# DoHoonKim8/halo2-lasso

Hardware: AMD Instinct MI355X
Metric: lasso_prove_time_ms (lower is better)
Workload: dtype u256 (BN254 Fr/Fq, 8x u32 Montgomery); 1 GPU; 2^24 AND Lasso lookup (32-bit operands, 4 chunks of 8+8 bits); lookups_per_proof=16777216, pcs=multilinear KZG (BN254), proof_bytes=64256, parallelism=1 GPU

## Files before the change

halo2-lasso_amd/_ffi.py:

```python
import ctypes as C
import os

_HERE = os.path.dirname(os.path.abspath(__file__))
LIB_PATH = os.path.join(_HERE, "liblasso_hip.so")

LH_OK = 0
LH_ERR_INVALID_SUMCHECK, LH_ERR_INVALID_PCS_PARAM, LH_ERR_INVALID_PCS_OPEN = -1, -2, -3
LH_ERR_INVALID_SNARK, LH_ERR_SERIALIZATION, LH_ERR_TRANSCRIPT, LH_ERR_DEVICE, LH_ERR_ARG = -4, -5, -6, -7, -8
LH_SC_EVALUATIONS, LH_SC_COEFFICIENTS = 0, 1
LH_SC_MAX_TERMS, LH_SC_MAX_FACTORS = 48, 4
LH_LASSO_MAX_CHUNKS, LH_LASSO_MAX_MEMORIES, LH_LASSO_MAX_TERMS = 8, 16, 16
LH_SUBTABLE_IDENTITY, LH_SUBTABLE_AND, LH_SUBTABLE_XOR, LH_SUBTABLE_OR, LH_SUBTABLE_EQ, LH_SUBTABLE_LTU = 0, 1, 2, 3, 4, 5
LH_SUBTABLE_CUSTOM_BASE, LH_SUBTABLE_CUSTOM_MAX, LH_SUBTABLE_CUSTOM_MAX_BITS = 0x100, 64, 20
LH_LASSO_NUM_PHASES = 9
LH_LOGUP_MAX_LOOKUPS, LH_LOGUP_MAX_WIDTH, LH_LOGUP_MAX_TABLE_VARS = 8, 8, 24
LH_LOGUP_COL_FR, LH_LOGUP_COL_U32 = 0, 1
LH_MEMCHECK_MAX_INIT_VARS = 24
LH_SPARK_MAX_DIMS, LH_SPARK_MAX_DIM_VARS = 3, 24
LH_BD_COLUMN_FR, LH_BD_COLUMN_U32 = 0, 1


class lh_fr(C.Structure):
    _fields_ = [("l", C.c_uint64 * 4)]

# ... 84 lines not shown


_AG_CB = C.CFUNCTYPE(C.c_int, C.c_void_p, C.c_void_p, C.c_void_p, C.c_size_t)
_AGD_CB = C.CFUNCTYPE(C.c_int, C.c_void_p, C.c_void_p, C.c_void_p, C.c_size_t, C.c_void_p)
LH_RCCL_UNIQUE_ID_BYTES = 128


class lh_comm(C.Structure):
    _fields_ = [("rank", C.c_int), ("size", C.c_int), ("user", C.c_void_p), ("all_gather", _AG_CB),
                ("all_gather_device", _AGD_CB)]


class lh_debug_sort_slab(C.Structure):
    _fields_ = [("d_keys_in", C.c_void_p), ("d_keys_out", C.c_void_p), ("d_vals_in", C.c_void_p), ("d_vals_out", C.c_void_p),
                ("n", C.c_size_t), ("bits", C.c_uint32), ("first_bit", C.c_uint32)]


class lh_debug_u32_args(C.Structure):
    _fields_ = [("d_cols", C.POINTER(C.c_void_p)), ("lens", C.POINTER(C.c_size_t)), ("w", C.POINTER(lh_fr)),
                ("count", C.c_size_t), ("d_weights", C.c_void_p), ("n", C.c_size_t),
                ("d_fr", C.POINTER(C.c_void_p)), ("w_fr", C.POINTER(lh_fr)), ("num_fr", C.c_size_t),
                ("r0", lh_fr), ("r1", lh_fr), ("d_out", C.c_void_p), ("out_host", C.POINTER(lh_fr)),
                ("taken", C.POINTER(C.c_int))]


LH_U32_OPS = ("inner_products_small", "inner_products_small_half", "inner_products_small_quads", "inner_products_quads",
              "lincomb_mixed", "lincomb_fold_small", "lincomb_bind2", "sc_round_u32_bind2", None,
              "quad_sums")


# ... 172 lines not shown
    "lh_hyrax_open": (C.c_int, [_P, _P, _SZ, _SZ, _P, _SZ, C.POINTER(lh_fr), C.POINTER(lh_transcript)]),
    "lh_hyrax_batch_open": (C.c_int, [_P, _P, _SZ, _SZ, _SZ, C.POINTER(_P), _SZ, C.POINTER(lh_fr), _SZ,
                                      C.POINTER(lh_evaluation), _SZ, C.POINTER(lh_transcript)]),
    "lh_hyrax_verify": (C.c_int, [_P, _SZ, _SZ, C.POINTER(lh_g1), C.POINTER(lh_fr), _SZ, C.POINTER(lh_fr),
                                  C.POINTER(lh_transcript)]),
    "lh_hyrax_batch_verify": (C.c_int, [_P, _SZ, _SZ, _SZ, C.POINTER(lh_g1), _SZ, C.POINTER(lh_fr), _SZ,
                                        C.POINTER(lh_evaluation), _SZ, C.POINTER(lh_transcript)]),
    "lh_debug_jit_source": (C.c_int, [C.POINTER(C.c_uint32), _SZ, C.c_uint32, C.c_uint32, C.c_int, C.c_char_p, _SZ,
                                      C.POINTER(_SZ)]),
    "lh_debug_sort_pairs": (C.c_int, [_P, C.c_int, C.POINTER(lh_debug_sort_slab), _SZ]),
    "lh_debug_lasso_counters": (C.c_int, [_P, C.POINTER(_P), _SZ, _SZ, _SZ, C.POINTER(_P), C.POINTER(_P), C.POINTER(_P),
                                          C.POINTER(_P)]),
    "lh_debug_sort_plan": (C.c_int, [_SZ, C.c_uint, C.c_int, C.POINTER(C.c_uint), C.POINTER(C.c_uint), C.POINTER(_SZ)]),
    "lh_debug_msm_plan": (C.c_int, [_SZ, C.POINTER(_SZ), C.POINTER(C.c_uint32), C.POINTER(C.c_uint32), C.c_int, C.c_int,
                                    C.POINTER(C.c_uint64), C.POINTER(_SZ)]),
    "lh_debug_u32_columns": (C.c_int, [_P, C.c_int, C.POINTER(lh_debug_u32_args)]),
    "lh_debug_lasso_subtable_read": (C.c_int, [_P, C.c_uint32, C.c_uint32, _P, _SZ, _P]),
    "lh_keccak_transcript_hash_io": (C.c_int, [C.POINTER(lh_transcript), C.POINTER(lh_hash_transcript)]),
    "lh_brakedown_setup": (C.c_int, [_P, _SZ, C.c_int, C.c_char_p, C.POINTER(_P)]),
    "lh_brakedown_derive": (C.c_int, [_SZ, C.c_int, C.POINTER(_P)]),
    "lh_brakedown_param_info": (C.c_int, [_P, C.POINTER(_SZ), C.POINTER(_SZ), C.POINTER(_SZ), C.POINTER(_SZ),
                                          C.POINTER(_SZ)]),
    "lh_brakedown_trim": (C.c_int, [_P, _SZ]),
    "lh_brakedown_param_free": (None, [_P]),
    "lh_brakedown_encode": (C.c_int, [_P, C.POINTER(lh_fr), C.POINTER(lh_fr)]),
    "lh_brakedown_commit": (C.c_int, [_P, _P, _P, _SZ, C.POINTER(_P)]),
    "lh_brakedown_batch_commit": (C.c_int, [_P, _P, C.POINTER(_P), _SZ, _SZ, C.POINTER(_P)]),
    "lh_brakedown_commit_columns": (C.c_int, [_P, _P, C.POINTER(_P), C.POINTER(C.c_int), C.POINTER(_SZ), _SZ, C.POINTER(_P)]),
    "lh_brakedown_comm_root": (C.c_int, [_P, C.c_char_p]),
    "lh_brakedown_comm_rows": (C.c_int, [_P, _P, _P]),
# ... 98 lines not shown
```

halo2-lasso_amd/csrc/capi.cpp:

```cpp
#include "host.hpp"
#include "brakedown.hpp"
#include <memory>

using namespace lh;

struct lh_ctx {
  Ctx c;
};
struct lh_srs {
  Srs s;
};
struct lh_mkzg_vp {
  VerifierParams* p;
};
struct lh_usrs {
  USrs s;
};
struct lh_zm_vp {
  ZmVerifierParams* p;
};
struct lh_ukzg_vp {
  UkzgVerifierParams* p;
};
struct lh_ipa_param {
// ... 2231 lines not shown
  NEED(out);
  NEED(num_subs);
  LH_REQUIRE(num_jobs >= 1 && num_jobs <= 48, LH_ERR_ARG, "debug msm plan: 1 .. 48 jobs");
  Ctx c;
  c.is_helper = helper != 0;
  std::vector<MsmJob> jobs;
  G1Affine second;
  for (size_t j = 0; j < num_jobs; j++) {
    LH_REQUIRE(bits[j] >= 1 && bits[j] <= (kinds[j] ? 32u : 254u), LH_ERR_ARG, "debug msm plan: bad width");
    MsmJob jb{nullptr, kinds[j] != 0, nullptr, n[j]};
    jb.known_bits = bits[j];
    if (kinds[j] >= 4) jb.pack_shift = kinds[j], jb.out_second = &second;
    jobs.push_back(jb);
  }
  *num_subs = msm_plan_shape(c, jobs.data(), num_jobs, via_prepare != 0, out);
  LH_CATCH
}

lh_status lh_debug_u32_columns(lh_ctx* ctx, int op, const lh_debug_u32_args* a) {
  LH_TRY NEED_CTX(ctx);
  NEED(a);
  Ctx& c = ctx->c;
  LH_REQUIRE((op >= LH_U32_INNER_PRODUCTS_SMALL && op <= LH_U32_SC_ROUND_BIND2) || op == LH_U32_QUAD_SUMS, LH_ERR_ARG,
             "debug u32 columns: unknown operation");
  LH_REQUIRE(a->n >= 1 && a->n < ((size_t)1 << 31), LH_ERR_ARG, "debug u32 columns: n must be in [1, 2^31)");
  const bool one_col = op == LH_U32_INNER_PRODUCTS_SMALL_QUADS || op == LH_U32_SC_ROUND_BIND2;
  const bool has_lens = op == LH_U32_INNER_PRODUCTS_QUADS || op == LH_U32_QUAD_SUMS || op == LH_U32_LINCOMB_MIXED ||
                        op == LH_U32_LINCOMB_FOLD_SMALL || op == LH_U32_LINCOMB_BIND2;
  const bool has_w = op == LH_U32_LINCOMB_MIXED || op == LH_U32_LINCOMB_FOLD_SMALL || op == LH_U32_LINCOMB_BIND2;
  const bool quads = op == LH_U32_INNER_PRODUCTS_SMALL_QUADS || op == LH_U32_INNER_PRODUCTS_QUADS || op == LH_U32_QUAD_SUMS ||
// ... 121 lines not shown
```

halo2-lasso_amd/csrc/dev.hpp:

```cpp
#pragma once
#include <hip/hip_runtime_api.h>
#include <stdint.h>
#include <stdarg.h>
#include <stdio.h>
#include <functional>
#include <memory>
#include <string>
#include <vector>
#include <utility>
#include <stdexcept>

#include "../../include/lasso_hip.h"
#include "ec.cuh"

namespace lh {

struct Error : std::exception {
  int code;
  std::string msg;
  Error(int c, std::string m) : code(c), msg(std::move(m)) {}
  const char* what() const noexcept override { return msg.c_str(); }
};

void set_last_error(const char* msg);
// ... 346 lines not shown
void k_lasso_rw_leaves(Ctx&, const uint32_t* dim, const uint32_t* e, const uint32_t* ts, size_t n,
                       const Fr& gamma, const Fr& gamma2, const Fr& tau, Fr* rs, Fr* ws);
void k_lasso_rw_leaves_up(Ctx&, const uint32_t* dim, const uint32_t* e, const uint32_t* ts, size_t n, const Fr& gamma,
                          const Fr& gamma2, const Fr& tau, Fr* rs, Fr* ws, Fr* rs_up, Fr* ws_up);
constexpr int LASSO_RW_BATCH_MAX = 8;
struct LassoRwBatch {
  const uint32_t *dim[LASSO_RW_BATCH_MAX], *e[LASSO_RW_BATCH_MAX], *ts[LASSO_RW_BATCH_MAX];
  Fr *rs[LASSO_RW_BATCH_MAX], *ws[LASSO_RW_BATCH_MAX], *rs_up[LASSO_RW_BATCH_MAX], *ws_up[LASSO_RW_BATCH_MAX];
};
void k_lasso_rw_leaves_batch(Ctx&, const LassoRwBatch& p, size_t num_memories, size_t n, bool up, const Fr& gamma,
                             const Fr& gamma2, const Fr& tau);
void k_lasso_if_leaves(Ctx&, int subtable, uint32_t chunk_bits, const uint32_t* final_cts, size_t m,
                       const Fr& gamma, const Fr& gamma2, const Fr& tau, Fr* init, Fr* fin, const uint32_t* tab = nullptr);
void k_or_u32(Ctx&, const uint32_t* const* cols, size_t count, size_t n, uint32_t* out_host);
void k_fill_u32(Ctx&, uint32_t* out, uint32_t value, size_t n);
void k_pack_u32(Ctx&, const uint32_t* a, const uint32_t* b, uint32_t shift, size_t n, uint32_t* out);
void k_delta_u32(Ctx&, const uint32_t* col, size_t len, size_t half, uint64_t offset, uint32_t* out_lo, uint32_t* out_hi);
void k_lasso_counters(Ctx&, const uint32_t* const* dims, size_t cc, size_t n, size_t m, uint32_t* const* read_ts,
                      uint32_t* const* final_cts, uint32_t* const* keep_sorted = nullptr, uint32_t* const* keep_index = nullptr);
void k_cs_partition(Ctx&, const uint32_t* const* dims, size_t cc, size_t n, size_t m, unsigned rho, unsigned j, unsigned hi_bits,
                    uint32_t* const* sidx, uint32_t* const* send, uint32_t* start_host, bool* bad_out);
void k_cs_rank(Ctx&, const uint32_t* const* recv, const size_t* n_recv, size_t cc, unsigned hi_bits, unsigned a_bits, size_t m_loc,
               uint32_t* const* ret, uint32_t* counts);
void k_cs_scatter(Ctx&, const uint32_t* const* back, const uint32_t* const* sidx, size_t cc, size_t n, uint32_t* const* read_ts);
void k_cs_final(Ctx&, const uint32_t* all_counts, size_t cc, size_t m, unsigned rho, size_t m_loc, uint32_t* const* final_cts);
void k_lasso_subtable_read(Ctx&, int subtable, uint32_t chunk_bits, const uint32_t* dim, size_t n, uint32_t* e,
                           const uint32_t* tab = nullptr);
struct LassoG {
  uint32_t num_terms;
  Fr coeff[LH_LASSO_MAX_TERMS];
  uint8_t nfac[LH_LASSO_MAX_TERMS];
// ... 294 lines not shown
  const uint32_t* keys_in;
  uint32_t* keys_out;
  const uint32_t* vals_in;
  uint32_t* vals_out;
  size_t n;
  unsigned bits;
  unsigned first_bit = 0;
};
void sort_pairs_u32(Ctx&, const uint32_t* keys_in, uint32_t* keys_out, const uint32_t* vals_in, uint32_t* vals_out, size_t n,
                    unsigned bits, unsigned first_bit = 0);
void sort_pairs_u32_batched(Ctx&, const SortSlab* slabs, size_t count);
void sort_pairs_u64(Ctx&, const uint64_t* keys_in, uint64_t* keys_out, const uint32_t* vals_in, uint32_t* vals_out, size_t n,
                    unsigned bits);
void sort_plan(size_t n, unsigned bits, size_t key_bytes, unsigned* passes, unsigned rb[8], size_t* temp_bytes);

struct MsmJob {
  const void* scalars;
  bool scalars_u32;
  const G1Affine* bases;
  size_t n;
  int derived_parent = -1;
  const uint32_t* d_table = nullptr;
  const uint32_t* d_order = nullptr;
  uint32_t table_in_bits = 0, table_out_bits = 0;
  const uint32_t* sorted_scalars = nullptr;
  const uint32_t* sorted_index = nullptr;
  uint32_t pack_shift = 0;
  G1Affine* out_second = nullptr;
  uint32_t known_bits = 0;
  const G1Affine* win_table = nullptr;
  uint32_t win_table_c = 0, win_table_W = 0;
};
constexpr uint32_t MSM_PACK_MAX_BITS = 20;
constexpr size_t MSM_PACK_MIN_POINTS_PER_BUCKET = 8;
Ctx& ctx_helper(Ctx&);
void open_precommit_cancel(Ctx&);
void open_precommit_release(Ctx&);
uint32_t msm_window_bits(size_t n);
void k_msm_window_table(Ctx&, const G1Affine* bases, size_t n, uint32_t cbits, uint32_t W, G1Affine* out);
bool msm_batch(Ctx&, const MsmJob* jobs, size_t num_jobs, G1Affine* out_host, const std::function<void()>* overlap = nullptr,
               const std::function<void(bool on_aux)>* acc_queued = nullptr);
struct MsmPrepared;
struct MsmPreparedDelete {
  void operator()(MsmPrepared*) const;
};
typedef std::unique_ptr<MsmPrepared, MsmPreparedDelete> MsmPreparedPtr;
// ... 8 lines not shown
```

halo2-lasso_amd/csrc/kernels_poly.hip:

```cpp
#include <hip/hip_runtime.h>
#include <string.h>
#include <algorithm>
#include "dev.hpp"
#include "ff_host.hpp"
#include "launch.cuh"
#include "reduce.cuh"
#include "resident.cuh"
#include "wide.cuh"

namespace lh {

__global__ void fr_from_u64_kernel(const uint64_t* __restrict__ in, size_t n, Fr* __restrict__ out) {
  GSTRIDE(i, n) out[i] = from_u64<FrParams>(in[i]);
}
__global__ void fr_from_u32_kernel(const uint32_t* __restrict__ in, size_t n, Fr* __restrict__ out) {
  GSTRIDE(i, n) out[i] = from_u64<FrParams>(in[i]);
}
__global__ void fr_to_repr_kernel(const Fr* __restrict__ in, size_t n, Fr* __restrict__ out) {
  GSTRIDE(i, n) out[i] = from_mont(in[i]);
}
__global__ void fr_from_repr_kernel(const Fr* __restrict__ in, size_t n, Fr* __restrict__ out) {
  GSTRIDE(i, n) out[i] = to_mont(in[i]);
}
void k_fr_from_u64(Ctx& c, const uint64_t* in, size_t n, Fr* out) {
// ... 1486 lines not shown
  GSTRIDE(i, half) {
    const uint64_t lo = i < len ? col[i] : 0u, hi = i + half < len ? col[i + half] : 0u;
    const uint64_t v = hi + offset - lo;
    if (out_hi) {
      out_lo[i] = (uint32_t)(v & 0xffffu);
      out_hi[i] = (uint32_t)(v >> 16);
    } else {
      out_lo[i] = (uint32_t)v;
    }
  }
}
void k_delta_u32(Ctx& c, const uint32_t* col, size_t len, size_t half, uint64_t offset, uint32_t* out_lo, uint32_t* out_hi) {
  if (half)
    hipLaunchKernelGGL(delta_u32_kernel, grid_for(half), 256, 0, c.stream, col, len, half, offset, out_lo, out_hi);
}
__global__ void pack_u32_kernel(const uint32_t* __restrict__ a, const uint32_t* __restrict__ b, uint32_t shift, size_t n,
                                uint32_t* __restrict__ out) {
  GSTRIDE(i, n) out[i] = a[i] | (b[i] << shift);
}
void k_pack_u32(Ctx& c, const uint32_t* a, const uint32_t* b, uint32_t shift, size_t n, uint32_t* out) {
  if (n) hipLaunchKernelGGL(pack_u32_kernel, grid_for(n), 256, 0, c.stream, a, b, shift, n, out);
}

__global__ void lasso_rw_leaves_kernel(const uint32_t* __restrict__ dim, const uint32_t* __restrict__ e,
                                       const uint32_t* __restrict__ ts, size_t n, Fr gamma_r, Fr gamma2_r, Fr one_r, Fr tau,
                                       Fr* __restrict__ rs, Fr* __restrict__ ws) {
  const Fr one = Fr::one();
  GSTRIDE(i, n) {
    Wide t = Wide::zero();
    wide_mac(t, gamma2_r, dim[i]);
    wide_mac(t, gamma_r, e[i]);
    wide_mac(t, one_r, ts[i]);
    Fr h = sub(wide_redc(t), tau);
    rs[i] = h;
    ws[i] = add(h, one);
  }
}
// ... 150 lines not shown
```

halo2-lasso_amd/csrc/lasso.cpp:

```cpp
#include <algorithm>
#include <chrono>
#include "host.hpp"

namespace lh {

static double now_ms() {
  using namespace std::chrono;
  return duration<double, std::milli>(steady_clock::now().time_since_epoch()).count();
}

void lasso_write_commitments(Transcript& tr, const std::vector<HG1>& comms, size_t chunks) {
  LH_REQUIRE(chunks >= 1 && comms.size() % chunks == 0 && comms.size() / chunks < 64, LH_ERR_ARG,
             "lasso: too many commitments for the identity mask");
  for (size_t k = 0; 63 * k < comms.size(); k++) {
    uint64_t mask = 0;
    for (size_t i = 0; i < 63 && 63 * k + i < comms.size(); i++)
      if (comms[63 * k + i].is_identity()) mask |= (uint64_t)1 << i;
    tr.write_field_element(HFr::from_u64(mask));
  }
  for (const HG1& cm : comms)
    if (!cm.is_identity()) tr.write_commitment(cm);
}

std::vector<HG1> lasso_read_commitments(Transcript& tr, size_t count, size_t chunks) {
// ... 449 lines not shown
    own++;
  }
  plan.second.assign(cc, HG1());
  std::vector<HG1>& second = plan.second;
  {
    std::vector<uint32_t>& ors = count_ors;
    std::vector<const uint32_t*> cols(fcs.begin(), fcs.end());
    const bool pack_on = c.opt.lasso_pack_ts != 0;
    if (!ors_known && pack_on && cc >= 2 && N >= ((size_t)1 << 12)) k_or_u32(c, cols.data(), cc, M, ors.data());
    for (size_t j = 0; j < cc; j++) {
      if (shared(j)) continue;
      const bool next = j + 1 < cc && !shared(j + 1);
      const uint32_t b0 = std::max(bit_length(ors[j]), 4u), b1 = next ? bit_length(ors[j + 1]) : 0;
      if (ors[j] && next && ors[j + 1] && b0 + b1 <= MSM_PACK_MAX_BITS &&
          N >= ((size_t)MSM_PACK_MIN_POINTS_PER_BUCKET << (b0 + b1))) {
        uint32_t* packed = c.arena.alloc_n<uint32_t>(N);
        k_pack_u32(c, rts[j], rts[j + 1], b0, N, packed);
        add_job(lay.read_ts(j), packed, true, N);
        jobs.back().known_bits = b0 + b1;
        jobs.back().pack_shift = b0;
        jobs.back().out_second = (G1Affine*)&second[j + 1];
        plan.second_of.push_back(j + 1);
        c.route.v[RouteStats::PACKED_TS]++;
        j++;
      } else {
        add_job(lay.read_ts(j), rts[j], true, N);
        jobs.back().known_bits = bit_length(ors[j]);
      }
    }
  }
  SubtableOrders& orders = *w.tables;
  for (size_t i = 0; i < alpha; i++)
    if (tb.memory_subtable[i] != LH_SUBTABLE_IDENTITY) {
      add_job(lay.E(i), E[i], true, N);
      bool derive = l <= 20 && tb.memory_subtable[i] != LH_SUBTABLE_EQ;
// ... 483 lines not shown
```

halo2-lasso_amd/csrc/msm.hip:

```cpp
#include <hip/hip_runtime.h>
#include <algorithm>
#include <exception>
#include <functional>
#include <thread>
#include <vector>
#include <mutex>
#include "dev.hpp"
#include "ff_host.hpp"

namespace lh {

constexpr int MSM_MAX_JOBS = 48;
constexpr uint32_t SENTINEL = 0xffffffffu;
constexpr uint32_t SKIP_IDX = 0x7fffffffu;

struct MsmJobDev {
  const void* scalars;
  const G1Affine* bases;
  uint32_t is_u32;
  uint32_t n;
  uint32_t c, W;
  uint32_t key_base;
  uint32_t entry_base;
  uint32_t win_stride;
  uint32_t is_signed;
  uint32_t seg_base;
  uint32_t seg_per_win;
  uint32_t seg_size;
  uint32_t win_base;
  uint32_t presorted;
// ... 3 lines not shown
  uint32_t share_base;
  uint32_t two_level;
  uint32_t grp_base;
  uint32_t sum_per_win;
  uint32_t merged;
};
constexpr uint32_t KEY_BLOCK_BITS = 10;
struct MsmPlanDev {
  int num_jobs;
  const uint8_t* job_of_block;
  MsmJobDev job[MSM_MAX_JOBS];
};

__global__ void msm_or_limbs_kernel(MsmPlanDev plan, uint32_t* __restrict__ or_out ) {
  const MsmJobDev& jb = plan.job[blockIdx.y];
  uint32_t acc[8];
#pragma unroll
  for (int k = 0; k < 8; k++) acc[k] = 0;
  if (jb.is_u32) {
    for (size_t i = (size_t)blockIdx.x * blockDim.x + threadIdx.x; i < jb.n; i += (size_t)gridDim.x * blockDim.x)
      acc[0] |= ((const uint32_t*)jb.scalars)[i];
  } else {
    for (size_t i = (size_t)blockIdx.x * blockDim.x + threadIdx.x; i < jb.n; i += (size_t)gridDim.x * blockDim.x) {
      Fr s = from_mont(((const Fr*)jb.scalars)[i]);
#pragma unroll
      for (int k = 0; k < 8; k++) acc[k] |= s.l[k];
    }
  }
  __shared__ uint32_t lds_or[8];
  if (threadIdx.x < 8) lds_or[threadIdx.x] = 0;
// ... 6 lines not shown
  }
  __syncthreads();
  if (threadIdx.x < 8 && lds_or[threadIdx.x]) atomicOr(&or_out[blockIdx.y * 8 + threadIdx.x], lds_or[threadIdx.x]);
}

__global__ void msm_presorted_kernel(uint32_t key_base, const uint32_t* __restrict__ sorted_scalars,
                                     const uint32_t* __restrict__ sorted_index, size_t n, uint32_t* __restrict__ skey,
                                     uint32_t* __restrict__ sidx) {
  for (size_t p = (size_t)blockIdx.x * blockDim.x + threadIdx.x; p < n; p += (size_t)gridDim.x * blockDim.x) {
    const uint32_t d = sorted_scalars[p];
    skey[p] = key_base + (d ? d - 1u : 0u);
    sidx[p] = d ? sorted_index[p] : SKIP_IDX;
  }
}

__global__ void msm_emit_kernel(MsmPlanDev plan, uint32_t* __restrict__ keys, uint32_t* __restrict__ vals) {
  const MsmJobDev& jb = plan.job[blockIdx.y];
  if (jb.presorted) return;
  const uint32_t c = jb.c, mask = (1u << c) - 1u;
  for (size_t i = (size_t)blockIdx.x * blockDim.x + threadIdx.x; i < jb.n; i += (size_t)gridDim.x * blockDim.x) {
    uint32_t limb[8];
#pragma unroll
    for (int k = 0; k < 8; k++) limb[k] = 0;
    if (jb.is_u32) {
      limb[0] = ((const uint32_t*)jb.scalars)[i];
    } else {
      Fr s = from_mont(((const Fr*)jb.scalars)[i]);
#pragma unroll
      for (int k = 0; k < 8; k++) limb[k] = s.l[k];
    }
    const int nlimbs = jb.is_u32 ? 1 : 8;
    uint64_t buf = 0;
    int have = 0;
    uint32_t w = 0;
    uint32_t carry = 0;
    const uint32_t half = 1u << (c - 1);
    auto emit = [&](uint32_t raw) {
      uint32_t d = raw + carry, neg = 0;
      if (jb.is_signed) {
// ... 435 lines not shown
namespace {
struct MsmSub {
  std::vector<size_t> idx;
  MsmPlanDev plan;
  std::vector<uint32_t> bits, sort_bits;
  std::vector<char> derived, slab;
  size_t num_derived = 0, max_entries = 0, small_entries = 0, max_n = 0, nbuckets = 0, nsegs = 0, nwins = 0, ngroups = 0, nblocks = 0;
  size_t nchunks = 0;
  uint32_t nshares = 0, K = 0, seg_size = 0;
  bool plain_reduce = false;
  double total_pts = 0, full_pts = 0;
  uint32_t *ukey = nullptr, *uidx = nullptr, *skey = nullptr, *sidx = nullptr, *lvl_cnt = nullptr, *ckey = nullptr;
  G1Xyzz *buckets = nullptr, *seg_out = nullptr, *seg_t = nullptr, *grp_out = nullptr, *cpt = nullptr;
  G1Xyzz* win_out = nullptr;
  uint8_t* h_tab = nullptr;
  std::vector<G1Xyzz> wins;
  size_t pin_bytes() const { return ((size_t)nshares * sizeof(G1Xyzz) + nblocks + 255) & ~(size_t)255; }
};

struct MsmShape {
  uint32_t c, W, sort_bits;
  size_t entries, buckets;
};
MsmShape msm_job_shape(const MsmJob& in, uint32_t bits, bool derived) {
  MsmShape s;
  s.c = pick_window(in.n ? in.n : 1, bits ? bits : 1);
  if (in.pack_shift) s.c = std::max<uint32_t>(bits, 4);
  const bool is_signed = !in.scalars_u32;
  if (is_signed && s.c < 2) s.c = 2;
  s.W = bits ? ((is_signed ? bits + 1 : bits) + s.c - 1) / s.c : 0;
  if (!in.n) s.W = 0;
  s.sort_bits = is_signed ? s.c - 1 : s.c;
// ... 63 lines not shown
      const uint32_t cw = pick_window(in.n, bits);
      est += ((size_t)(bits + cw) / cw) << (in.scalars_u32 ? cw : cw - 1);
    }
    const uint32_t forced = (uint32_t)knob(Knob::MSM_SEG);
    seg_size = forced ? forced : est <= ((size_t)1 << 18) ? 4u : est <= ((size_t)1 << 20) ? 8u : 16u;
    if (whole) seg_size = whole->seg_size;
    s.seg_size = seg_size;
  }
  uint32_t key = 0, seg = 0, win = 0;
  const int slab_log = (int)knob(Knob::MSM_SLAB_LOG);
  for (size_t j = 0; j < nj; j++) {
    const MsmJob& in = jobs[s.idx[j]];
    MsmJobDev& jd = plan.job[j];
    const uint32_t bits = s.bits[j];
    jd.scalars = in.scalars;
    jd.is_u32 = in.scalars_u32 ? 1 : 0;
    jd.n = (uint32_t)in.n;
    jd.bases = in.bases;
    if (s.derived[j]) jd.n = 0;
    jd.c = pick_window(in.n ? in.n : 1, bits ? bits : 1);
    jd.pack_shift = 0;
    if (in.pack_shift) {
      LH_REQUIRE(in.scalars_u32 && in.out_second && in.pack_shift >= 4 && bits <= MSM_PACK_MAX_BITS && !s.derived[j],
                 LH_ERR_ARG, "msm: bad packed job");
      jd.pack_shift = in.pack_shift;
      jd.c = std::max<uint32_t>(bits, 4);
    }
    jd.is_signed = in.scalars_u32 ? 0 : 1;
    if (jd.is_signed && jd.c < 2) jd.c = 2;
    jd.W = bits ? ((jd.is_signed ? bits + 1 : bits) + jd.c - 1) / jd.c : 0;
    if (!in.n) jd.W = 0;
// ... 61 lines not shown
  uint32_t nsplit = 1;
  {
    uint32_t max_spw = 1;
    for (size_t j = 0; j < nj; j++)
      if (plan.job[j].W && plan.job[j].sum_per_win < 16384) max_spw = std::max(max_spw, plan.job[j].sum_per_win);
    while (nsplit < 32 && max_spw / nsplit > 1024 && s.nwins * nsplit * 2 <= 4096) nsplit *= 2;
  }
  s.nshares = 0;
  for (size_t j = 0; j < nj; j++) {
    MsmJobDev& jd = plan.job[j];
    jd.nsplit = jd.sum_per_win >= 16384 ? std::max<uint32_t>(nsplit, 32u) : nsplit;
    jd.share_base = s.nshares;
    s.nshares += jd.red_W * jd.nsplit;
  }
  s.nblocks = (s.nbuckets >> KEY_BLOCK_BITS) + 1;
  s.total_pts = s.full_pts = 0;
  for (size_t j = 0; j < nj; j++) s.total_pts += plan.job[j].n, s.full_pts += plan.job[j].is_u32 ? 0 : plan.job[j].n;
  const size_t me = s.max_entries;
  s.K = me > ((size_t)1 << 26) ? 128 : me > ((size_t)1 << 25) ? 64 : me > ((size_t)1 << 23) ? 32 : me > ((size_t)1 << 21) ? 16 : me > ((size_t)1 << 18) ? 8 : 4;
  if (whole) s.K = whole->K;
  s.nchunks = (me + s.K - 1) / s.K;
  s.wins.assign(s.nshares, G1Xyzz::identity());
}

static void msm_sub_alloc(Ctx& c, MsmSub& s, uint8_t* pin_at) {
  s.ukey = c.arena.alloc_n<uint32_t>(s.max_entries);
  s.uidx = c.arena.alloc_n<uint32_t>(s.max_entries);
  s.skey = c.arena.alloc_n<uint32_t>(s.max_entries + 256);
  s.sidx = c.arena.alloc_n<uint32_t>(s.max_entries + 256);
  s.buckets = c.arena.alloc_n<G1Xyzz>(s.nbuckets);
  s.seg_out = c.arena.alloc_n<G1Xyzz>(s.nsegs);
  s.seg_t = s.ngroups ? c.arena.alloc_n<G1Xyzz>(s.nsegs) : nullptr;
  s.grp_out = s.ngroups ? c.arena.alloc_n<G1Xyzz>(s.ngroups) : nullptr;
  s.lvl_cnt = c.arena.alloc_n<uint32_t>(64);
  s.ckey = c.arena.alloc_n<uint32_t>(s.nchunks);
  s.cpt = c.arena.alloc_n<G1Xyzz>(s.nchunks);
  s.win_out = (G1Xyzz*)pin_at;
  s.h_tab = pin_at + (size_t)s.nshares * sizeof(G1Xyzz);
}

static void msm_sub_entries(Ctx& c, const MsmJob* jobs, MsmSub& s) {
  const size_t nj = s.idx.size();
  MsmPlanDev& plan = s.plan;
  {
    for (size_t j = 0; j < nj; j++) {
      const size_t b0 = plan.job[j].key_base >> KEY_BLOCK_BITS;
      const size_t b1 = j + 1 < nj ? plan.job[j + 1].key_base >> KEY_BLOCK_BITS : s.nblocks;
      for (size_t b = b0; b < b1; b++) s.h_tab[b] = (uint8_t)j;
    }
    uint8_t* d_tab = c.arena.alloc_n<uint8_t>(s.nblocks);
    LH_HIP(hipMemcpyAsync(d_tab, s.h_tab, s.nblocks, hipMemcpyHostToDevice, c.stream));
    plan.job_of_block = d_tab;
  }
  for (size_t j = 0; j < nj; j++) c.route.v[RouteStats::WIN_TABLE_JOBS] += plan.job[j].merged ? 1 : 0;
  LH_HIP(hipMemsetAsync(s.lvl_cnt, 0, 64 * sizeof(uint32_t), c.stream));
  LH_HIP(hipMemsetAsync(s.buckets, 0, s.nbuckets * sizeof(G1Xyzz), c.stream));
  unsigned key_bits = 1;
  while (((size_t)1 << key_bits) <= s.nbuckets) key_bits++;
  {
    ProfScope ps(c, "msm_digits", 32.0 * s.full_pts + 4.0 * (s.total_pts - s.full_pts) + 8.0 * s.max_entries, s.full_pts,
                 s.total_pts);
    dim3 g((unsigned)std::min<size_t>((s.max_n + 255) / 256, 2048), (unsigned)nj);
    hipLaunchKernelGGL(msm_emit_kernel, g, dim3(256), 0, c.stream, plan, s.ukey, s.uidx);
  }
  {
    ProfScope ps(c, "msm_sort", 32.0 * s.max_entries, 0, (double)s.max_entries);
    std::vector<SortSlab> sorts;
    if (s.small_entries) sorts.push_back(SortSlab{s.ukey, s.skey, s.uidx, s.sidx, s.small_entries, key_bits});
    for (size_t j = 0; j < nj; j++) {
      if (!s.slab[j]) continue;
      const MsmJobDev& jd = plan.job[j];
      if (jd.presorted) {
        const MsmJob& in = jobs[s.idx[j]];
        hipLaunchKernelGGL(msm_presorted_kernel, dim3((unsigned)std::min<size_t>((jd.n + 255) / 256, 4096)), dim3(256), 0,
                           c.stream, jd.key_base, in.sorted_scalars, in.sorted_index, (size_t)jd.n, s.skey + jd.entry_base,
                           s.sidx + jd.entry_base);
        continue;
      }
      if (jd.merged) {
// ... 123 lines not shown
  });
}

namespace {
struct MsmChunk {
  size_t base = 0, nj = 0, total_entries = 0;
  std::vector<MsmSub> subs;
  bool waited = false;
};
}
struct MsmPrepared {
  MsmChunk first;
};
void MsmPreparedDelete::operator()(MsmPrepared* p) const { delete p; }

static void msm_chunk_prepare(Ctx& c, const MsmJob* jobs, size_t base, size_t nj, MsmChunk& ch, bool queue = true) {
  ch.base = base, ch.nj = nj;
  {
    std::vector<uint32_t> job_bits(nj, 32);
    {
      MsmPlanDev or_plan;
      or_plan.num_jobs = (int)nj;
      or_plan.job_of_block = nullptr;
      bool any_fr = false, any_unknown = false;
      size_t max_n0 = 0;
      for (size_t j = 0; j < nj; j++) {
        const MsmJob& in = jobs[base + j];
        LH_REQUIRE(in.n < ((size_t)1 << 31), LH_ERR_ARG, "msm: too many points");
        memset(&or_plan.job[j], 0, sizeof(MsmJobDev));
        or_plan.job[j].scalars = in.scalars;
        or_plan.job[j].is_u32 = in.scalars_u32 ? 1 : 0;
        or_plan.job[j].n = in.known_bits ? 0u : (uint32_t)in.n;
// ... 56 lines not shown
      msm_plan_sub(c, jobs, s, subs.size() == 2 ? &whole : nullptr);
      total_entries += s.max_entries, pin_total += s.pin_bytes();
    }
    ch.total_entries = total_entries;
    if (total_entries == 0) return;
    if (subs.size() == 2 && (!subs[0].max_entries || !subs[1].max_entries)) {
      subs.assign(1, whole);
      pin_total = subs[0].pin_bytes();
    }
    if (!queue) return;
    uint8_t* pin_base = (uint8_t*)c.pin(pin_total);
    for (MsmSub& s : subs) {
      msm_sub_alloc(c, s, pin_base);
      pin_base += s.pin_bytes();
    }
    for (MsmSub& s : subs) msm_sub_entries(c, jobs, s);
  }
}

static void msm_chunk_run(Ctx& c, const MsmJob* jobs, size_t num_jobs, G1Affine* out_host, MsmChunk& ch,
                          const std::function<void()>* overlap, bool& overlap_done, const std::function<void(bool)>* acc_queued) {
  const size_t base = ch.base, nj = ch.nj;
  std::vector<MsmSub>& subs = ch.subs;
  {
    if (ch.total_entries == 0) {
      for (size_t j = 0; j < nj; j++) {
        memset(&out_host[base + j], 0, sizeof(G1Affine));
        if (jobs[base + j].out_second) memset(jobs[base + j].out_second, 0, sizeof(G1Affine));
      }
      if (acc_queued) (*acc_queued)(false);
      return;
// ... 216 lines not shown
```

halo2-lasso_amd/csrc/open_columns.cpp:

```cpp
#include <algorithm>
#include <functional>
#include <chrono>
#include <memory>
#include <thread>
#include "open_columns.hpp"

namespace lh {

void column_shape(Ctx& c, const std::vector<SmallPoly>& cols, const std::vector<char>& zero, size_t n,
                         size_t num_vars, size_t cut, ColumnPlan& plan) {
  const size_t K = cols.size(), half_top = n >> 1;
  std::vector<uint32_t>& ors = plan.ors;
  ors.assign(K, 0);
  std::map<size_t, std::vector<size_t>> by_len;
  for (size_t k = 0; k < K; k++) {
    if (cols[k].len <= (half_top >> 1) || zero[k]) continue;
    if (cols[k].bits) ors[k] = cols[k].bits >= 32 ? 0xffffffffu : (1u << cols[k].bits) - 1u;
    else by_len[cols[k].len].push_back(k);
  }
  for (const auto& grp : by_len) {
    std::vector<const uint32_t*> ptrs;
    for (size_t k : grp.second) ptrs.push_back(cols[k].ptr);
    std::vector<uint32_t> o(ptrs.size(), 0);
    k_or_u32(c, ptrs.data(), ptrs.size(), grp.first, o.data());
// ... 19 lines not shown
  const size_t depth = plan.depth;
  const std::vector<uint32_t>& ors = plan.ors;
  std::vector<MsmJob>& jobs = plan.jobs;
  plan.levels.assign(depth, ColLevel());
  size_t num_seconds = 0;
  for (size_t d = 0; d < depth; d++) num_seconds += cols.size() << d;
  plan.seconds.assign(num_seconds, HG1());
  size_t next_second = 0;
  for (size_t d = 0; d < depth; d++) {
    ColLevel& cl = plan.levels[d];
    cl.level = num_vars - 1 - d;
    const size_t half = (size_t)1 << (cl.level - lsh);
    const G1Affine* bases = level_bases(cl.level);
    struct Narrow {
      uint32_t bits;
      uint32_t* col;
      size_t k, sidx;
    };
    std::vector<Narrow> narrow;
    for (size_t sidx = 0; sidx < ((size_t)1 << d); sidx++) {
      const size_t off_idx = sidx << (cl.level + 1 - lsh);
      for (size_t k = 0; k < cols.size(); k++) {
        const SmallPoly& sp = cols[k];
        if (zero[k] || sp.len <= off_idx) continue;
        const uint32_t* sub = sp.ptr + off_idx;
        const size_t sub_len = std::min(sp.len - off_idx, half << 1);
        if (sub_len <= half) {
          jobs.push_back(MsmJob{sub, true, bases, sub_len});
          if (sp.bits) jobs.back().known_bits = sp.bits;
          cl.terms.push_back(ColTerm{jobs.size() - 1, false, k, sidx, -1});
          continue;
// ... 3 lines not shown
        const uint64_t off = (uint64_t)1 << b;
        cl.offsets.push_back(ColOffset{k, sidx, off});
        cl.need_sum = true;
        if (b + 1 > 32) {
          uint32_t* lo = c.arena.alloc_n<uint32_t>(half);
          uint32_t* hi = c.arena.alloc_n<uint32_t>(half);
          k_delta_u32(c, sub, sub_len, half, off, lo, hi);
          jobs.push_back(MsmJob{lo, true, bases, half});
          jobs.back().known_bits = 16;
          cl.terms.push_back(ColTerm{jobs.size() - 1, false, k, sidx, 1});
          jobs.push_back(MsmJob{hi, true, bases, half});
          jobs.back().known_bits = b + 1 - 16;
          cl.terms.push_back(ColTerm{jobs.size() - 1, false, k, sidx, 65536});
          continue;
        }
        uint32_t* dcol = c.arena.alloc_n<uint32_t>(half);
        k_delta_u32(c, sub, sub_len, half, off, dcol, nullptr);
        if (b + 1 <= MSM_PACK_MAX_BITS - 4) {
          narrow.push_back(Narrow{b + 1, dcol, k, sidx});
        } else {
          jobs.push_back(MsmJob{dcol, true, bases, half});
          jobs.back().known_bits = b + 1;
          cl.terms.push_back(ColTerm{jobs.size() - 1, false, k, sidx, 1});
        }
      }
    }
    std::stable_sort(narrow.begin(), narrow.end(), [](const Narrow& x, const Narrow& y) { return x.bits < y.bits; });
    for (size_t i = 0; i < narrow.size(); i++) {
      const Narrow& x = narrow[i];
      const uint32_t shift = std::max(x.bits, 4u);
      if (i + 1 < narrow.size() && shift + narrow[i + 1].bits <= MSM_PACK_MAX_BITS &&
          half >= ((size_t)MSM_PACK_MIN_POINTS_PER_BUCKET << (shift + narrow[i + 1].bits))) {
        const Narrow& y = narrow[i + 1];
        uint32_t* packed = c.arena.alloc_n<uint32_t>(half);
        k_pack_u32(c, x.col, y.col, shift, half, packed);
        MsmJob jb{packed, true, bases, half};
        jb.pack_shift = shift;
        jb.known_bits = shift + y.bits;
        jb.out_second = (G1Affine*)&plan.seconds[next_second++];
        jobs.push_back(jb);
        cl.terms.push_back(ColTerm{jobs.size() - 1, false, x.k, x.sidx, 1});
        cl.terms.push_back(ColTerm{jobs.size() - 1, true, y.k, y.sidx, 1});
        i++;
      } else {
        jobs.push_back(MsmJob{x.col, true, bases, half});
        jobs.back().known_bits = x.bits;
        cl.terms.push_back(ColTerm{jobs.size() - 1, false, x.k, x.sidx, 1});
      }
    }
    if (cl.need_sum) {
      std::lock_guard<std::mutex> lock(srs_cache_mu);
      std::map<size_t, HG1>& sums = sharded ? srs.shard_level_sums : srs.level_sums;
      auto it = sums.find(cl.level);
      if (it != sums.end()) {
        cl.base_sum = it->second;
      } else {
        uint32_t* ones = c.arena.alloc_n<uint32_t>(half);
        k_fill_u32(c, ones, 1u, half);
        jobs.push_back(MsmJob{ones, true, bases, half});
        jobs.back().known_bits = 1;
        cl.sum_job = jobs.size() - 1;
// ... 186 lines not shown
```

include/lasso_hip.h:

```cpp
#ifndef LASSO_HIP_H
#define LASSO_HIP_H

#include <stddef.h>
#include <stdint.h>

#ifdef __cplusplus
extern "C" {
#endif

typedef struct { uint64_t l[4]; } lh_fr;
typedef struct { uint64_t x[4], y[4]; } lh_g1;

typedef int lh_status;
#define LH_OK 0
#define LH_ERR_INVALID_SUMCHECK (-1)
#define LH_ERR_INVALID_PCS_PARAM (-2)
#define LH_ERR_INVALID_PCS_OPEN (-3)
#define LH_ERR_INVALID_SNARK (-4)
#define LH_ERR_SERIALIZATION (-5)
#define LH_ERR_TRANSCRIPT (-6)
#define LH_ERR_DEVICE (-7)
#define LH_ERR_ARG (-8)

typedef struct lh_ctx lh_ctx;
// ... 543 lines not shown
  uint32_t* d_vals_out;
  size_t n;
  uint32_t bits, first_bit;
} lh_debug_sort_slab;
lh_status lh_debug_sort_pairs(lh_ctx*, int key_bytes, const lh_debug_sort_slab* slabs, size_t count);
lh_status lh_debug_lasso_counters(lh_ctx*, const uint32_t* const* d_dims, size_t num_cols, size_t n, size_t m,
                                  uint32_t* const* d_read_ts, uint32_t* const* d_final_cts, uint32_t* const* d_keep_sorted,
                                  uint32_t* const* d_keep_index);
lh_status lh_debug_memcheck_witness(lh_ctx*, const lh_memcheck_trace*, size_t num_vars, size_t mem_vars, const uint32_t* init,
                                    uint32_t* d_rt, uint32_t* d_fv, uint32_t* d_ft, uint32_t* d_m, int* out_bad);
lh_status lh_debug_spark_e(lh_ctx*, size_t num_vars, size_t dim_vars, size_t num_dims, const uint32_t* const* d_dims,
                           const lh_fr* d_val, const lh_fr* point, lh_fr* const* d_E, lh_fr* out_value);
lh_status lh_debug_sort_plan(size_t n, unsigned bits, int key_bytes, unsigned* passes, unsigned rb[8], size_t* temp_bytes);
lh_status lh_debug_msm_plan(size_t num_jobs, const size_t* n, const uint32_t* bits, const uint32_t* kinds, int helper, int via_prepare,
                            uint64_t* out, size_t* num_subs);

enum {
  LH_U32_INNER_PRODUCTS_SMALL = 0,
  LH_U32_INNER_PRODUCTS_SMALL_HALF = 1,
  LH_U32_INNER_PRODUCTS_SMALL_QUADS = 2,
  LH_U32_INNER_PRODUCTS_QUADS = 3,
  LH_U32_LINCOMB_MIXED = 4,
  LH_U32_LINCOMB_FOLD_SMALL = 5,
  LH_U32_LINCOMB_BIND2 = 6,
  LH_U32_SC_ROUND_BIND2 = 7,
  LH_U32_QUAD_SUMS = 9
};
typedef struct lh_debug_u32_args {
  const uint32_t* const* d_cols;
  const size_t* lens;
// ... 31 lines not shown
```

Baseline: 53.67 ms.

## Fuse u32 pack and delta computation into MSM digit emission kernel

Instead of materialising packed (a | b<<shift) and delta (hi+off-lo) u32 columns with separate kernels and arena buffers before the MSM, jobs now carry a small expression descriptor that the MSM emit kernel evaluates on the fly. This removes extra kernel launches and the full write and read of intermediate columns for read-timestamp packing and column-opening deltas. It adds a per-job expression struct copied to the device, skips these jobs in the OR-limb width scan (so they must promise known_bits), and adds a debug entry point for batch MSM.

```diff
diff --git a/halo2-lasso_amd/_ffi.py b/halo2-lasso_amd/_ffi.py
--- a/halo2-lasso_amd/_ffi.py
+++ b/halo2-lasso_amd/_ffi.py
@@ -122,6 +122,15 @@
 class lh_debug_sort_slab(C.Structure):
     _fields_ = [("d_keys_in", C.c_void_p), ("d_keys_out", C.c_void_p), ("d_vals_in", C.c_void_p), ("d_vals_out", C.c_void_p),
                 ("n", C.c_size_t), ("bits", C.c_uint32), ("first_bit", C.c_uint32)]
+
+
+class lh_debug_msm_term(C.Structure):
+    _fields_ = [("d_col", C.c_void_p), ("len", C.c_size_t), ("half", C.c_size_t), ("off", C.c_uint64)]
+
+
+class lh_debug_msm_job(C.Structure):
+    _fields_ = [("d_scalars", C.c_void_p), ("n", C.c_size_t), ("known_bits", C.c_uint32), ("pack_shift", C.c_uint32),
+                ("expr_terms", C.c_uint32), ("expr", lh_debug_msm_term * 2)]
 
 
 class lh_debug_u32_args(C.Structure):
@@ -324,6 +333,7 @@
     "lh_debug_sort_plan": (C.c_int, [_SZ, C.c_uint, C.c_int, C.POINTER(C.c_uint), C.POINTER(C.c_uint), C.POINTER(_SZ)]),
     "lh_debug_msm_plan": (C.c_int, [_SZ, C.POINTER(_SZ), C.POINTER(C.c_uint32), C.POINTER(C.c_uint32), C.c_int, C.c_int,
                                     C.POINTER(C.c_uint64), C.POINTER(_SZ)]),
+    "lh_debug_msm_batch": (C.c_int, [_P, _P, _SZ, C.POINTER(lh_debug_msm_job), _SZ, C.POINTER(lh_g1)]),
     "lh_debug_u32_columns": (C.c_int, [_P, C.c_int, C.POINTER(lh_debug_u32_args)]),
     "lh_debug_lasso_subtable_read": (C.c_int, [_P, C.c_uint32, C.c_uint32, _P, _SZ, _P]),
     "lh_keccak_transcript_hash_io": (C.c_int, [C.POINTER(lh_transcript), C.POINTER(lh_hash_transcript)]),
diff --git a/halo2-lasso_amd/csrc/capi.cpp b/halo2-lasso_amd/csrc/capi.cpp
--- a/halo2-lasso_amd/csrc/capi.cpp
+++ b/halo2-lasso_amd/csrc/capi.cpp
@@ -2269,6 +2269,44 @@
     jobs.push_back(jb);
   }
   *num_subs = msm_plan_shape(c, jobs.data(), num_jobs, via_prepare != 0, out);
+  LH_CATCH
+}
+
+lh_status lh_debug_msm_batch(lh_ctx* ctx, const lh_g1* d_bases, size_t num_bases, const lh_debug_msm_job* jobs, size_t num_jobs,
+                             lh_g1* out) {
+  LH_TRY NEED_CTX(ctx);
+  NEED(d_bases);
+  NEED_N(jobs, num_jobs);
+  NEED_N(out, num_jobs);
+  LH_REQUIRE(num_jobs >= 1 && num_jobs <= 48, LH_ERR_ARG, "debug msm batch: 1 .. 48 jobs");
+  std::vector<MsmJob> v;
+  for (size_t j = 0; j < num_jobs; j++) {
+    const lh_debug_msm_job& in = jobs[j];
+    LH_REQUIRE(in.n >= 1 && in.n <= num_bases && in.n < ((size_t)1 << 31), LH_ERR_ARG, "debug msm batch: n must be in [1, num_bases]");
+    LH_REQUIRE(in.known_bits <= 32 && in.expr_terms <= 2, LH_ERR_ARG, "debug msm batch: bad width or expression");
+    LH_REQUIRE((in.d_scalars != nullptr) == (in.expr_terms == 0), LH_ERR_ARG, "debug msm batch: a column or an expression");
+    if (in.pack_shift)
+      LH_REQUIRE(in.pack_shift >= 4 && in.known_bits > in.pack_shift && in.known_bits <= MSM_PACK_MAX_BITS, LH_ERR_ARG,
+                 "debug msm batch: bad packed job");
+    MsmJob jb{in.d_scalars, true, (const G1Affine*)d_bases, in.n};
+    jb.known_bits = in.known_bits, jb.pack_shift = in.pack_shift;
+    jb.expr_terms = in.expr_terms;
+    for (uint32_t t = 0; t < in.expr_terms; t++) {
+      const lh_debug_msm_term& x = in.expr[t];
+      LH_REQUIRE(x.d_col != nullptr && x.half < ((size_t)1 << 31), LH_ERR_ARG, "debug msm batch: bad expression operand");
+      jb.expr[t].col = x.d_col, jb.expr[t].len = x.len, jb.expr[t].half = x.half, jb.expr[t].off = x.off;
+    }
+    v.push_back(jb);
+  }
+  std::vector<G1Affine> first(num_jobs), second(num_jobs);
+  memset((void*)second.data(), 0, num_jobs * sizeof(G1Affine));
+  for (size_t j = 0; j < num_jobs; j++)
+    if (v[j].pack_shift) v[j].out_second = &second[j];
+  msm_batch(ctx->c, v.data(), num_jobs, first.data());
+  for (size_t j = 0; j < num_jobs; j++) {
+    memcpy(&out[2 * j], &first[j], sizeof(lh_g1));
+    memcpy(&out[2 * j + 1], &second[j], sizeof(lh_g1));
+  }
   LH_CATCH
 }
 
diff --git a/halo2-lasso_amd/csrc/dev.hpp b/halo2-lasso_amd/csrc/dev.hpp
--- a/halo2-lasso_amd/csrc/dev.hpp
+++ b/halo2-lasso_amd/csrc/dev.hpp
@@ -384,7 +384,6 @@
                        const Fr& gamma, const Fr& gamma2, const Fr& tau, Fr* init, Fr* fin, const uint32_t* tab = nullptr);
 void k_or_u32(Ctx&, const uint32_t* const* cols, size_t count, size_t n, uint32_t* out_host);
 void k_fill_u32(Ctx&, uint32_t* out, uint32_t value, size_t n);
-void k_pack_u32(Ctx&, const uint32_t* a, const uint32_t* b, uint32_t shift, size_t n, uint32_t* out);
 void k_delta_u32(Ctx&, const uint32_t* col, size_t len, size_t half, uint64_t offset, uint32_t* out_lo, uint32_t* out_hi);
 void k_lasso_counters(Ctx&, const uint32_t* const* dims, size_t cc, size_t n, size_t m, uint32_t* const* read_ts,
                       uint32_t* const* final_cts, uint32_t* const* keep_sorted = nullptr, uint32_t* const* keep_index = nullptr);
@@ -709,6 +708,11 @@
                     unsigned bits);
 void sort_plan(size_t n, unsigned bits, size_t key_bytes, unsigned* passes, unsigned rb[8], size_t* temp_bytes);
 
+struct MsmTerm {
+  const uint32_t* col = nullptr;
+  size_t len = 0, half = 0;
+  uint64_t off = 0;
+};
 struct MsmJob {
   const void* scalars;
   bool scalars_u32;
@@ -725,6 +729,8 @@
   uint32_t known_bits = 0;
   const G1Affine* win_table = nullptr;
   uint32_t win_table_c = 0, win_table_W = 0;
+  uint32_t expr_terms = 0;
+  MsmTerm expr[2];
 };
 constexpr uint32_t MSM_PACK_MAX_BITS = 20;
 constexpr size_t MSM_PACK_MIN_POINTS_PER_BUCKET = 8;
diff --git a/halo2-lasso_amd/csrc/kernels_poly.hip b/halo2-lasso_amd/csrc/kernels_poly.hip
--- a/halo2-lasso_amd/csrc/kernels_poly.hip
+++ b/halo2-lasso_amd/csrc/kernels_poly.hip
@@ -1524,13 +1524,6 @@
   if (half)
     hipLaunchKernelGGL(delta_u32_kernel, grid_for(half), 256, 0, c.stream, col, len, half, offset, out_lo, out_hi);
 }
-__global__ void pack_u32_kernel(const uint32_t* __restrict__ a, const uint32_t* __restrict__ b, uint32_t shift, size_t n,
-                                uint32_t* __restrict__ out) {
-  GSTRIDE(i, n) out[i] = a[i] | (b[i] << shift);
-}
-void k_pack_u32(Ctx& c, const uint32_t* a, const uint32_t* b, uint32_t shift, size_t n, uint32_t* out) {
-  if (n) hipLaunchKernelGGL(pack_u32_kernel, grid_for(n), 256, 0, c.stream, a, b, shift, n, out);
-}
 
 __global__ void lasso_rw_leaves_kernel(const uint32_t* __restrict__ dim, const uint32_t* __restrict__ e,
                                        const uint32_t* __restrict__ ts, size_t n, Fr gamma_r, Fr gamma2_r, Fr one_r, Fr tau,
diff --git a/halo2-lasso_amd/csrc/lasso.cpp b/halo2-lasso_amd/csrc/lasso.cpp
--- a/halo2-lasso_amd/csrc/lasso.cpp
+++ b/halo2-lasso_amd/csrc/lasso.cpp
@@ -487,11 +487,12 @@
       const uint32_t b0 = std::max(bit_length(ors[j]), 4u), b1 = next ? bit_length(ors[j + 1]) : 0;
       if (ors[j] && next && ors[j + 1] && b0 + b1 <= MSM_PACK_MAX_BITS &&
           N >= ((size_t)MSM_PACK_MIN_POINTS_PER_BUCKET << (b0 + b1))) {
-        uint32_t* packed = c.arena.alloc_n<uint32_t>(N);
-        k_pack_u32(c, rts[j], rts[j + 1], b0, N, packed);
-        add_job(lay.read_ts(j), packed, true, N);
+        add_job(lay.read_ts(j), nullptr, true, N);
         jobs.back().known_bits = b0 + b1;
         jobs.back().pack_shift = b0;
+        jobs.back().expr_terms = 2;
+        jobs.back().expr[0].col = rts[j], jobs.back().expr[0].len = N;
+        jobs.back().expr[1].col = rts[j + 1], jobs.back().expr[1].len = N;
         jobs.back().out_second = (G1Affine*)&second[j + 1];
         plan.second_of.push_back(j + 1);
         c.route.v[RouteStats::PACKED_TS]++;
diff --git a/halo2-lasso_amd/csrc/msm.hip b/halo2-lasso_amd/csrc/msm.hip
--- a/halo2-lasso_amd/csrc/msm.hip
+++ b/halo2-lasso_amd/csrc/msm.hip
@@ -14,6 +14,15 @@
 constexpr uint32_t SENTINEL = 0xffffffffu;
 constexpr uint32_t SKIP_IDX = 0x7fffffffu;
 
+struct MsmTermDev {
+  const uint32_t* col;
+  uint32_t len, half;
+  uint64_t off;
+};
+struct MsmExprDev {
+  MsmTermDev t[2];
+  uint32_t terms, shift;
+};
 struct MsmJobDev {
   const void* scalars;
   const G1Affine* bases;
@@ -47,6 +56,7 @@
 
 __global__ void msm_or_limbs_kernel(MsmPlanDev plan, uint32_t* __restrict__ or_out ) {
   const MsmJobDev& jb = plan.job[blockIdx.y];
+  if (jb.is_u32 == 2) return;
   uint32_t acc[8];
 #pragma unroll
   for (int k = 0; k < 8; k++) acc[k] = 0;
@@ -83,15 +93,27 @@
   }
 }
 
+__device__ __forceinline__ uint32_t msm_term_value(const MsmTermDev& t, size_t i) {
+  const uint32_t lo = i < t.len ? t.col[i] : 0u;
+  if (!t.half) return lo;
+  const uint32_t hi = i + t.half < t.len ? t.col[i + t.half] : 0u;
+  return (uint32_t)((uint64_t)hi + t.off - (uint64_t)lo);
+}
+
 __global__ void msm_emit_kernel(MsmPlanDev plan, uint32_t* __restrict__ keys, uint32_t* __restrict__ vals) {
   const MsmJobDev& jb = plan.job[blockIdx.y];
   if (jb.presorted) return;
   const uint32_t c = jb.c, mask = (1u << c) - 1u;
+  MsmExprDev ex = {};
+  if (jb.is_u32 == 2) ex = *(const MsmExprDev*)jb.scalars;
   for (size_t i = (size_t)blockIdx.x * blockDim.x + threadIdx.x; i < jb.n; i += (size_t)gridDim.x * blockDim.x) {
     uint32_t limb[8];
 #pragma unroll
     for (int k = 0; k < 8; k++) limb[k] = 0;
-    if (jb.is_u32) {
+    if (jb.is_u32 == 2) {
+      limb[0] = msm_term_value(ex.t[0], i);
+      if (ex.terms == 2) limb[0] |= msm_term_value(ex.t[1], i) << ex.shift;
+    } else if (jb.is_u32) {
       limb[0] = ((const uint32_t*)jb.scalars)[i];
     } else {
       Fr s = from_mont(((const Fr*)jb.scalars)[i]);
@@ -557,8 +579,13 @@
   G1Xyzz *buckets = nullptr, *seg_out = nullptr, *seg_t = nullptr, *grp_out = nullptr, *cpt = nullptr;
   G1Xyzz* win_out = nullptr;
   uint8_t* h_tab = nullptr;
+  size_t num_expr = 0;
+  MsmExprDev *h_expr = nullptr, *d_expr = nullptr;
   std::vector<G1Xyzz> wins;
-  size_t pin_bytes() const { return ((size_t)nshares * sizeof(G1Xyzz) + nblocks + 255) & ~(size_t)255; }
+  size_t tab_bytes() const { return (nblocks + 15) & ~(size_t)15; }
+  size_t pin_bytes() const {
+    return ((size_t)nshares * sizeof(G1Xyzz) + tab_bytes() + num_expr * sizeof(MsmExprDev) + 255) & ~(size_t)255;
+  }
 };
 
 struct MsmShape {
@@ -652,7 +679,7 @@
     MsmJobDev& jd = plan.job[j];
     const uint32_t bits = s.bits[j];
     jd.scalars = in.scalars;
-    jd.is_u32 = in.scalars_u32 ? 1 : 0;
+    jd.is_u32 = in.scalars_u32 ? (in.expr_terms ? 2 : 1) : 0;
     jd.n = (uint32_t)in.n;
     jd.bases = in.bases;
     if (s.derived[j]) jd.n = 0;
@@ -744,6 +771,8 @@
     s.nshares += jd.red_W * jd.nsplit;
   }
   s.nblocks = (s.nbuckets >> KEY_BLOCK_BITS) + 1;
+  s.num_expr = 0;
+  for (size_t j = 0; j < nj; j++) s.num_expr += plan.job[j].is_u32 == 2 ? 1 : 0;
   s.total_pts = s.full_pts = 0;
   for (size_t j = 0; j < nj; j++) s.total_pts += plan.job[j].n, s.full_pts += plan.job[j].is_u32 ? 0 : plan.job[j].n;
   const size_t me = s.max_entries;
@@ -767,9 +796,11 @@
   s.cpt = c.arena.alloc_n<G1Xyzz>(s.nchunks);
   s.win_out = (G1Xyzz*)pin_at;
   s.h_tab = pin_at + (size_t)s.nshares * sizeof(G1Xyzz);
-}
-
-static void msm_sub_entries(Ctx& c, const MsmJob* jobs, MsmSub& s) {
+  s.h_expr = (MsmExprDev*)(s.h_tab + s.tab_bytes());
+  s.d_expr = s.num_expr ? c.arena.alloc_n<MsmExprDev>(s.num_expr) : nullptr;
+}
+
+static void msm_sub_digits(Ctx& c, const MsmJob* jobs, MsmSub& s) {
   const size_t nj = s.idx.size();
   MsmPlanDev& plan = s.plan;
   {
@@ -782,17 +813,37 @@
     LH_HIP(hipMemcpyAsync(d_tab, s.h_tab, s.nblocks, hipMemcpyHostToDevice, c.stream));
     plan.job_of_block = d_tab;
   }
+  if (s.num_expr) {
+    size_t k = 0;
+    for (size_t j = 0; j < nj; j++) {
+      if (plan.job[j].is_u32 != 2) continue;
+      const MsmJob& in = jobs[s.idx[j]];
+      MsmExprDev& e = s.h_expr[k];
+      memset(&e, 0, sizeof(e));
+      e.terms = in.expr_terms, e.shift = in.pack_shift;
+      for (uint32_t t = 0; t < in.expr_terms; t++) {
+        const MsmTerm& x = in.expr[t];
+        e.t[t] = MsmTermDev{x.col, (uint32_t)std::min(x.len, x.half + in.n), (uint32_t)x.half, x.off};
+      }
+      plan.job[j].scalars = s.d_expr + k++;
+    }
+    LH_HIP(hipMemcpyAsync(s.d_expr, s.h_expr, s.num_expr * sizeof(MsmExprDev), hipMemcpyHostToDevice, c.stream));
+  }
   for (size_t j = 0; j < nj; j++) c.route.v[RouteStats::WIN_TABLE_JOBS] += plan.job[j].merged ? 1 : 0;
   LH_HIP(hipMemsetAsync(s.lvl_cnt, 0, 64 * sizeof(uint32_t), c.stream));
   LH_HIP(hipMemsetAsync(s.buckets, 0, s.nbuckets * sizeof(G1Xyzz), c.stream));
-  unsigned key_bits = 1;
-  while (((size_t)1 << key_bits) <= s.nbuckets) key_bits++;
   {
     ProfScope ps(c, "msm_digits", 32.0 * s.full_pts + 4.0 * (s.total_pts - s.full_pts) + 8.0 * s.max_entries, s.full_pts,
                  s.total_pts);
     dim3 g((unsigned)std::min<size_t>((s.max_n + 255) / 256, 2048), (unsigned)nj);
     hipLaunchKernelGGL(msm_emit_kernel, g, dim3(256), 0, c.stream, plan, s.ukey, s.uidx);
   }
+}
+static void msm_sub_sort(Ctx& c, const MsmJob* jobs, MsmSub& s) {
+  const size_t nj = s.idx.size();
+  MsmPlanDev& plan = s.plan;
+  unsigned key_bits = 1;
+  while (((size_t)1 << key_bits) <= s.nbuckets) key_bits++;
   {
     ProfScope ps(c, "msm_sort", 32.0 * s.max_entries, 0, (double)s.max_entries);
     std::vector<SortSlab> sorts;
@@ -946,8 +997,19 @@
 };
 void MsmPreparedDelete::operator()(MsmPrepared* p) const { delete p; }
 
+static void msm_check_expr(const MsmJob& in) {
+  if (!in.expr_terms) return;
+  LH_REQUIRE(in.known_bits != 0, LH_ERR_ARG, "msm: an expression job must promise its width (known_bits)");
+  LH_REQUIRE(in.scalars_u32 && !in.scalars && in.expr_terms <= 2 && (in.expr_terms == 2) == (in.pack_shift != 0) &&
+                 in.derived_parent < 0 && !in.sorted_scalars && !in.sorted_index,
+             LH_ERR_ARG, "msm: bad expression job");
+  for (uint32_t t = 0; t < in.expr_terms; t++)
+    LH_REQUIRE((in.expr[t].col || !in.n) && in.expr[t].half < ((size_t)1 << 31), LH_ERR_ARG, "msm: bad expression operand");
+}
+
 static void msm_chunk_prepare(Ctx& c, const MsmJob* jobs, size_t base, size_t nj, MsmChunk& ch, bool queue = true) {
   ch.base = base, ch.nj = nj;
+  for (size_t j = 0; j < nj; j++) msm_check_expr(jobs[base + j]);
   {
     std::vector<uint32_t> job_bits(nj, 32);
     {
@@ -1034,7 +1096,7 @@
       msm_sub_alloc(c, s, pin_base);
       pin_base += s.pin_bytes();
     }
-    for (MsmSub& s : subs) msm_sub_entries(c, jobs, s);
+    for (MsmSub& s : subs) msm_sub_digits(c, jobs, s), msm_sub_sort(c, jobs, s);
   }
 }
 
diff --git a/halo2-lasso_amd/csrc/open_columns.cpp b/halo2-lasso_amd/csrc/open_columns.cpp
--- a/halo2-lasso_amd/csrc/open_columns.cpp
+++ b/halo2-lasso_amd/csrc/open_columns.cpp
@@ -57,7 +57,7 @@
     const G1Affine* bases = level_bases(cl.level);
     struct Narrow {
       uint32_t bits;
-      uint32_t* col;
+      MsmTerm diff;
       size_t k, sidx;
     };
     std::vector<Narrow> narrow;
@@ -91,13 +91,14 @@
           cl.terms.push_back(ColTerm{jobs.size() - 1, false, k, sidx, 65536});
           continue;
         }
-        uint32_t* dcol = c.arena.alloc_n<uint32_t>(half);
-        k_delta_u32(c, sub, sub_len, half, off, dcol, nullptr);
+        MsmTerm diff;
+        diff.col = sub, diff.len = sub_len, diff.half = half, diff.off = off;
         if (b + 1 <= MSM_PACK_MAX_BITS - 4) {
-          narrow.push_back(Narrow{b + 1, dcol, k, sidx});
+          narrow.push_back(Narrow{b + 1, diff, k, sidx});
         } else {
-          jobs.push_back(MsmJob{dcol, true, bases, half});
+          jobs.push_back(MsmJob{nullptr, true, bases, half});
           jobs.back().known_bits = b + 1;
+          jobs.back().expr_terms = 1, jobs.back().expr[0] = diff;
           cl.terms.push_back(ColTerm{jobs.size() - 1, false, k, sidx, 1});
         }
       }
@@ -109,9 +110,8 @@
       if (i + 1 < narrow.size() && shift + narrow[i + 1].bits <= MSM_PACK_MAX_BITS &&
           half >= ((size_t)MSM_PACK_MIN_POINTS_PER_BUCKET << (shift + narrow[i + 1].bits))) {
         const Narrow& y = narrow[i + 1];
-        uint32_t* packed = c.arena.alloc_n<uint32_t>(half);
-        k_pack_u32(c, x.col, y.col, shift, half, packed);
-        MsmJob jb{packed, true, bases, half};
+        MsmJob jb{nullptr, true, bases, half};
+        jb.expr_terms = 2, jb.expr[0] = x.diff, jb.expr[1] = y.diff;
         jb.pack_shift = shift;
         jb.known_bits = shift + y.bits;
         jb.out_second = (G1Affine*)&plan.seconds[next_second++];
@@ -120,8 +120,9 @@
         cl.terms.push_back(ColTerm{jobs.size() - 1, true, y.k, y.sidx, 1});
         i++;
       } else {
-        jobs.push_back(MsmJob{x.col, true, bases, half});
+        jobs.push_back(MsmJob{nullptr, true, bases, half});
         jobs.back().known_bits = x.bits;
+        jobs.back().expr_terms = 1, jobs.back().expr[0] = x.diff;
         cl.terms.push_back(ColTerm{jobs.size() - 1, false, x.k, x.sidx, 1});
       }
     }
diff --git a/include/lasso_hip.h b/include/lasso_hip.h
--- a/include/lasso_hip.h
+++ b/include/lasso_hip.h
@@ -581,6 +581,19 @@
 lh_status lh_debug_sort_plan(size_t n, unsigned bits, int key_bytes, unsigned* passes, unsigned rb[8], size_t* temp_bytes);
 lh_status lh_debug_msm_plan(size_t num_jobs, const size_t* n, const uint32_t* bits, const uint32_t* kinds, int helper, int via_prepare,
                             uint64_t* out, size_t* num_subs);
+typedef struct lh_debug_msm_term {
+  const uint32_t* d_col;
+  size_t len, half;
+  uint64_t off;
+} lh_debug_msm_term;
+typedef struct lh_debug_msm_job {
+  const uint32_t* d_scalars;
+  size_t n;
+  uint32_t known_bits, pack_shift, expr_terms;
+  lh_debug_msm_term expr[2];
+} lh_debug_msm_job;
+lh_status lh_debug_msm_batch(lh_ctx*, const lh_g1* d_bases, size_t num_bases, const lh_debug_msm_job* jobs, size_t num_jobs,
+                             lh_g1* out);
 
 enum {
   LH_U32_INNER_PRODUCTS_SMALL = 0,
```

After: 53.86 ms. No clear change (+0.4%).
